# microsoft/M3P

Hardware: AMD Instinct MI355X
Metric: pre-train samples/sec (whole node), 12L/768d seq=128+36 (higher is better)
Workload: dtype bf16; 1 GPU; cfg2: 12L/768d/12h, 36 regions + 128 tokens, V=250002, 19 MLM targets/seq + ITM BCE, dropout 0.10, adam_inverse_sqrt + clip 5; per_gpu_batch=256, global_batch=256, seq_len=164, parallelism=dp1, prewarm_steps=36

## Files before the change

include/m3p_hip.h:

```cpp
#ifndef M3P_HIP_H
#define M3P_HIP_H

#include <stddef.h>
#include <stdint.h>

#ifdef __cplusplus
extern "C" {
#endif

#define M3P_API __attribute__((visibility("default")))

#define M3P_OK 0
#define M3P_EINVAL (-1)
#define M3P_ENOTIMPL (-2)
#define M3P_ENOMEM (-3)

M3P_API const char* m3p_version(void);


enum {
  M3P_EPI_NONE = 0,
  M3P_EPI_BIAS = 1,
  M3P_EPI_BIAS_GELU = 2,
  M3P_EPI_BIAS_DROP_RES = 3,
// ... 36 lines not shown
                            int M, int N, int K, int epilogue, const M3PEpilogue* ep, void* stream);

M3P_API int m3p_quant_fp8(const void* src, int ld_src, void* dst, int ld_dst, int rows, int cols, const float* scale,
                          float* amax, int bf8, void* stream);

M3P_API int m3p_quant_fp8_batch(const long long* desc, int n_desc, int blocks_per_matrix, void* stream);

M3P_API int m3p_gemm_nt_streamk_f32(const void* A, int lda, const void* W, int ldw, float* C, int ldc,
                                    int M, int N, int K, float alpha, void* stream);
M3P_API int m3p_gemm_nn_streamk_f32(const void* A, int lda, const void* W, int ldw, int k_valid, float* C,
                                    int ldc, int M, int N, int K, float alpha, void* stream);
M3P_API int m3p_gemm_nn_w4_f32(const void* A, int lda, const void* W, int ldw, float* C, int ldc, int M, int N, int K, float alpha,
                               void* workspace, size_t workspace_bytes, void* stream);

M3P_API size_t m3p_gemm_wgrad_workspace_bytes(void);
M3P_API int m3p_gemm_wgrad_bf16(const void* dY, int lddy, const void* X, int ldx, float* dW, int lddw,
                                int M, int N, int K, float alpha, void* workspace, size_t workspace_bytes,
                                void* stream);
M3P_API int m3p_gemm_wgrad_store_bf16(const void* dY, int lddy, const void* X, int ldx, float* dW, int lddw, int M, int N, int K,
                                      float alpha, void* workspace, size_t workspace_bytes, void* stream);
M3P_API int m3p_gemm_wgrad_pair_bf16(const void* dYa, int lddya, const void* Xa, int ldxa, float* dWa, int lddwa, int Na, int Ka,
                                     const void* dYb, int lddyb, const void* Xb, int ldxb, float* dWb, int lddwb, int Nb, int Kb,
                                     int M, float alpha, void* workspace, size_t workspace_bytes, void* stream);


M3P_API int m3p_layernorm_fwd(const void* x, const float* gamma, const float* beta, const uint8_t* rowmask,
                              void* y, float* mean, float* rstd, int rows, int d, float eps, void* stream);

M3P_API int m3p_layernorm_bwd(const void* dy_a, const void* dy_b, const void* x, const float* gamma,
                              const float* mean, const float* rstd, const uint8_t* rowmask,
                              void* dx, void* dx_drop, float* dgamma, float* dbeta, float* dbias_drop,
                              int rows, int d, uint32_t seed, uint32_t thresh24, float inv_keep, void* stream);
M3P_API int m3p_layernorm_bwd_rows(const void* dy_a, const void* dy_b, const void* x, const float* gamma,
                                   const float* mean, const float* rstd, const uint8_t* rowmask,
                                   void* dx, void* dx_drop, float* dgamma, float* dbeta, float* dbias_drop,
                                   int rows, int d, uint32_t seed, uint32_t thresh24, float inv_keep,
                                   const int32_t* rng_rows, void* stream);


M3P_API int m3p_attn_fwd(const void* qkv, const int32_t* keylen, void* ctx, float* lse, uint64_t* keepmask,
                         int B, int S, int H, int dh, uint32_t seed, uint32_t thresh24, float inv_keep,
                         void* stream);

M3P_API int m3p_attn_bwd(const void* qkv, const int32_t* keylen, const void* ctx, const void* dctx,
                         const float* lse, const uint64_t* keepmask, void* dqkv, float* dbias_qkv, int B, int S,
                         int H, int dh, float qscale, uint32_t seed, uint32_t thresh24, float inv_keep,
// ... 194 lines not shown
```

m3p_amd/csrc/gemm.hip:

```cpp
#include <mutex>
#include <type_traits>
#include "common.hpp"
#include "../../include/m3p_hip.h"
#include <hip/amd_detail/amd_hip_unsafe_atomics.h>

static int g_variant = 1;
extern "C" void m3p_debug_set_variant(int v) { g_variant = (v == 2 || v == 6) ? v : 1; }

namespace {

constexpr int BK = 64;
constexpr int ROWB = BK * 2;

#define M3P_DSR(dst, addr, off) asm volatile("ds_read_b128 %0, %1 offset:" #off : "=v"(dst) : "v"(addr))
#define M3P_TR(dst, addr, off) asm volatile("ds_read_b64_tr_b16 %0, %1 offset:" #off : "=v"(dst) : "v"(addr))
#define M3P_WAIT_LGKM(N) do { __builtin_amdgcn_sched_barrier(0); asm volatile("s_waitcnt lgkmcnt(" #N ")" ::: "memory"); __builtin_amdgcn_sched_barrier(0); } while (0)
#define M3P_WAIT_VM(N) do { __builtin_amdgcn_sched_barrier(0); asm volatile("s_waitcnt vmcnt(" #N ")" ::: "memory"); __builtin_amdgcn_sched_barrier(0); } while (0)
#define M3P_BAR() do { __builtin_amdgcn_s_barrier(); asm volatile("" ::: "memory"); __builtin_amdgcn_sched_barrier(0); } while (0)

__device__ __forceinline__ int xcd_slot(int nwg) {
  const int per_xcd = nwg >> 3;
  return (blockIdx.x & 7) * per_xcd + (blockIdx.x >> 3);
}
__device__ __forceinline__ int strip_width(int tiles_n, int from, int width) {
// ... 1647 lines not shown
      }
#pragma unroll
      for (int i = 0; i < 8; ++i)
#pragma unroll
        for (int j = 0; j < 4; ++j) acc[i][j] = f32x4{0.f, 0.f, 0.f, 0.f};
      if (more1) {
        read_w(nxt * STAGE, fw);
        read_a(Q0{}, nxt * STAGE, fa0);
        M3P_WAIT_LGKM(0);
      }
    }
  }
  if ((EPI == M3P_EPI_DGELU || EPI == M3P_EPI_MUL) && ep.colsum && csum_nw >= 0) flush_csum();
}


struct WgCursor {
  int c, t, mt, len;
};
struct WgradProblem {
  const bf16* dY; const bf16* X; float* dW;
  int lddy, ldx, lddw, tiles_i, tiles_j;
};

template <bool W_KN>
__global__ __launch_bounds__(512)
void gemm_nt_streamk_kernel(const bf16* __restrict__ A, int lda, const bf16* __restrict__ W, int ldw,
                            float* __restrict__ Cf, int ldc, int M, int N, int K, float alpha,
                            int tiles_m, int tiles_n, int CHUNK, int k_valid) {
  constexpr int BM = 256, BN = 128, NWAVES = 8;
  constexpr int A_BYTES = BM * ROWB, B_BYTES = BN * ROWB, STAGE = A_BYTES + B_BYTES;
  extern __shared__ __attribute__((aligned(16))) char smem[];
  const int tid = threadIdx.x, lane = tid & 63;
  const int wid = __builtin_amdgcn_readfirstlane(tid >> 6);
  const int ntile = tiles_m * tiles_n;
  const int nk = K / BK;
  const long long total_all = (long long)ntile * nk;
  const int nwg = gridDim.x;
  const int slot = xcd_slot(nwg);
  const long long share = (total_all + nwg - 1) / nwg;
  const long long g0l = share * slot;
  if (g0l >= total_all) return;
  const int total = (int)((g0l + share <= total_all ? g0l + share : total_all) - g0l);

  auto locate = [&](long long g) {
    WgCursor cu;
// ... 885 lines not shown
    return M3P_ENOTIMPL;
  return launch_wgrad_w4<true>(A, lda, W, ldw, C, ldc, K, M, N, alpha, workspace, workspace_bytes, stream, nullptr);
}

int m3p_gemm_wgrad_pair_bf16(const void* dYa, int lddya, const void* Xa, int ldxa, float* dWa, int lddwa, int Na, int Ka,
                             const void* dYb, int lddyb, const void* Xb, int ldxb, float* dWb, int lddwb, int Nb, int Kb,
                             int M, float alpha, void* workspace, size_t workspace_bytes, void* stream) {
  if (M <= 0 || Na <= 0 || Ka <= 0 || Nb <= 0 || Kb <= 0) return M3P_EINVAL;
  const bool pair = wgrad_w4_ok(M, Na, Ka, lddya, ldxa, dYa, Xa) && wgrad_w4_ok(M, Nb, Kb, lddyb, ldxb, dYb, Xb) &&
                    workspace && workspace_bytes >= m3p_gemm_wgrad_workspace_bytes() && (((uintptr_t)workspace & 15) == 0) &&
                    (lddwa % 4) == 0 && (lddwb % 4) == 0 && (((uintptr_t)dWa | (uintptr_t)dWb) & 15) == 0 &&
                    lddwa >= Ka && lddwb >= Kb &&
                    (long long)((Na / 256) * (Ka / 256) + (Nb / 256) * (Kb / 256)) * 2 <= num_cus();
  if (!pair) {
    int rc = m3p_gemm_wgrad_bf16(dYa, lddya, Xa, ldxa, dWa, lddwa, M, Na, Ka, alpha, workspace, workspace_bytes, stream);
    if (rc != M3P_OK) return rc;
    return m3p_gemm_wgrad_bf16(dYb, lddyb, Xb, ldxb, dWb, lddwb, M, Nb, Kb, alpha, workspace, workspace_bytes, stream);
  }
  if (lddya < Na || ldxa < Ka || lddyb < Nb || ldxb < Kb) return M3P_EINVAL;
  WgradProblem pb = {(const bf16*)dYb, (const bf16*)Xb, dWb, lddyb, ldxb, lddwb, Nb / 256, Kb / 256};
  return launch_wgrad_w4<>(dYa, lddya, Xa, ldxa, dWa, lddwa, M, Na, Ka, alpha, workspace, workspace_bytes, stream, &pb);
}

int m3p_gemm_wgrad_store_bf16(const void* dY, int lddy, const void* X, int ldx, float* dW, int lddw, int M, int N, int K,
                              float alpha, void* workspace, size_t workspace_bytes, void* stream) {
  if (M <= 0 || N <= 0 || K <= 0 || (lddy % 8) != 0 || (ldx % 8) != 0 || !dW || lddw < K) return M3P_EINVAL;
  if (lddy < N || ldx < K || ((uintptr_t)dY & 15) || ((uintptr_t)X & 15)) return M3P_EINVAL;
  if (!wgrad_w4_ok(M, N, K, lddy, ldx, dY, X)) return M3P_ENOTIMPL;
  return launch_wgrad_w4<>(dY, lddy, X, ldx, dW, lddw, M, N, K, alpha, workspace, workspace_bytes, stream, nullptr, true);
}

int m3p_gemm_wgrad_bf16(const void* dY, int lddy, const void* X, int ldx, float* dW, int lddw, int M, int N, int K,
                        float alpha, void* workspace, size_t workspace_bytes, void* stream) {
  if (M <= 0 || N <= 0 || K <= 0 || (lddy % 8) != 0 || (ldx % 8) != 0 || !dW || lddw < K) return M3P_EINVAL;
  if (lddy < ((N + 7) / 8) * 8 || ldx < ((K + 7) / 8) * 8) return M3P_EINVAL;
  if (((uintptr_t)dY & 15) || ((uintptr_t)X & 15)) return M3P_EINVAL;
  const int plan = wgrad_plan(M, N, K, wgrad_w4_ok(M, N, K, lddy, ldx, dY, X));
  if (plan == M3P_KERN_WGRAD_W4_CHUNKS || plan == M3P_KERN_WGRAD_W4_TILES) {
    return launch_wgrad_w4<>(dY, lddy, X, ldx, dW, lddw, M, N, K, alpha, workspace, workspace_bytes, stream, nullptr);
  }
  if (plan == M3P_KERN_WGRAD_RING) {
    const int ti = (N + WR_I - 1) / WR_I, tj = (K + WR_J - 1) / WR_J;
    const size_t lds = 3 * WR_STAGE;
    if (int rc = set_max_lds<gemm_wgrad_ring_kernel>(lds)) return rc;
    const int grid = num_cus();
    const int nmt = M / BK;
// ... 26 lines not shown
```

m3p_amd/csrc/gemm_wgrad_w4.hpp:

```cpp
template <bool YROWS>
__global__ __launch_bounds__(256)
void gemm_wgrad_w4_kernel(const bf16* __restrict__ dY_a, int lddy_a, const bf16* __restrict__ X_a, int ldx_a,
                          float* __restrict__ dW_a, int lddw_a, int M, int N, int K, float alpha,
                          int tiles_i, int tiles_j_a, int WR_CHUNK, float* __restrict__ ws, int* __restrict__ ws_tile,
                          int overwrite, WgradProblem pb) {
  const bf16* dY = dY_a;
  const bf16* X = X_a;
  float* dW = dW_a;
  int lddy = lddy_a, ldx = ldx_a, lddw = lddw_a, tiles_j = tiles_j_a;
  int tile_id0 = 0;
  constexpr int TI = 256, TJ = 256, KT = 64;
  constexpr int ROWB = 512;
  constexpr int Y_BYTES = KT * ROWB, STAGE = 2 * Y_BYTES;
  extern __shared__ __attribute__((aligned(16))) char smem[];
  const int tid = threadIdx.x, lane = tid & 63;
  const int wid = __builtin_amdgcn_readfirstlane(tid >> 6);
  const int ntile_a = tiles_i * tiles_j_a;
  const int ntile = ntile_a + pb.tiles_i * pb.tiles_j;
  const int nmt = M / KT;
  const long long total_all = (long long)ntile * nmt;
  const int nwg = gridDim.x;
  const int slot = xcd_slot(nwg);
  const bool rr = (WR_CHUNK == 0);
  if (ws && tid == 0) ws_tile[slot] = -1;
  int total, seg_tile, seg_m0, seg_len;
  if (rr) {
    const int my_tiles = (ntile > slot) ? (ntile - slot + nwg - 1) / nwg : 0;
    if (my_tiles == 0) return;
    total = my_tiles * nmt;
    seg_tile = slot; seg_m0 = 0; seg_len = nmt;
  } else {
    const int C = max(nwg / ntile, 1);
    if (slot >= C * ntile) return;
    const int c = slot / ntile;
    seg_tile = slot - c * ntile;
    if (seg_tile >= ntile_a) {
      dY = pb.dY; X = pb.X; dW = pb.dW; lddy = pb.lddy; ldx = pb.ldx; lddw = pb.lddw; tiles_j = pb.tiles_j;
      seg_tile -= ntile_a;
      tile_id0 = ntile_a;
    }
    seg_m0 = (int)((long long)c * nmt / C);
    seg_len = (int)((long long)(c + 1) * nmt / C) - seg_m0;
    total = seg_len;
    if (total <= 0) return;
  }
  (void)total_all;
  auto locate = [&](int) {
    WgCursor cu;
    cu.c = 0; cu.t = seg_tile; cu.mt = 0; cu.len = seg_len;
// ... 128 lines not shown
  asm volatile("" ::: "memory");
#pragma unroll
  for (int c = 0; c < 8; ++c) {
    WG_YRD(c, 0, 0);
    WG_TR2(xl[c], xh[c], x_addr[0][c], 0);
  }
  M3P_WAIT_LGKM(0);
#pragma unroll
  for (int c = 0; c < 8; ++c) { yf0[c] = yfrag(c); xf0[c] = frag(xl[c], xh[c]); }

  WgCursor cc = locate(g0);
  bool first = true;
  int n_seg = 0;
  auto kstep = [&](auto stage_c, int step) {
    if (first) wktile(std::true_type{}, stage_c);
    else wktile(std::false_type{}, stage_c);
    first = false;

    const bool last_of_tile = (cc.mt + 1 == cc.len) || (step + 1 == total);
    if (last_of_tile) {
      asm volatile("s_nop 15\n\ts_nop 15" ::: "memory");
      const int ti = cc.t / tiles_j, tj = cc.t - ti * tiles_j;
      float* dbase = dW + (size_t)(ti * TI + wi * 128 + fg * 4) * lddw + tj * TJ + wj * 128 + ft;
      const bool to_ws = (ws != nullptr) && !rr && n_seg == 0 && (step + 1 == total);
      if (to_ws) {
        asm volatile("s_waitcnt vmcnt(0)" ::: "memory");
        __builtin_amdgcn_s_barrier();
        asm volatile("" ::: "memory");
      }
#pragma nounroll
      for (int bb = 0; bb < 8; ++bb) {
        const int b = to_ws ? bb : ((bb + slot) & 7);
        float v[32];
#define WG_RD8(B)                                                                                   \
  _Pragma("unroll") for (int q = 0; q < 32; ++q) v[q] = 0.f;                                        \
  asm volatile("v_accvgpr_read_b32 %0, a[(" #B ")*32+0]\n\tv_accvgpr_read_b32 %1, a[(" #B ")*32+1]\n\t"   \
               "v_accvgpr_read_b32 %2, a[(" #B ")*32+2]\n\tv_accvgpr_read_b32 %3, a[(" #B ")*32+3]\n\t"   \
               "v_accvgpr_read_b32 %4, a[(" #B ")*32+4]\n\tv_accvgpr_read_b32 %5, a[(" #B ")*32+5]\n\t"   \
               "v_accvgpr_read_b32 %6, a[(" #B ")*32+6]\n\tv_accvgpr_read_b32 %7, a[(" #B ")*32+7]"       \
               : "=v"(v[0]), "=v"(v[1]), "=v"(v[2]), "=v"(v[3]), "=v"(v[4]), "=v"(v[5]), "=v"(v[6]), "=v"(v[7]));   \
  asm volatile("v_accvgpr_read_b32 %0, a[(" #B ")*32+8]\n\tv_accvgpr_read_b32 %1, a[(" #B ")*32+9]\n\t"   \
               "v_accvgpr_read_b32 %2, a[(" #B ")*32+10]\n\tv_accvgpr_read_b32 %3, a[(" #B ")*32+11]\n\t" \
               "v_accvgpr_read_b32 %4, a[(" #B ")*32+12]\n\tv_accvgpr_read_b32 %5, a[(" #B ")*32+13]\n\t" \
               "v_accvgpr_read_b32 %6, a[(" #B ")*32+14]\n\tv_accvgpr_read_b32 %7, a[(" #B ")*32+15]"     \
               : "=v"(v[8]), "=v"(v[9]), "=v"(v[10]), "=v"(v[11]), "=v"(v[12]), "=v"(v[13]), "=v"(v[14]), "=v"(v[15])); \
  asm volatile("v_accvgpr_read_b32 %0, a[(" #B ")*32+16]\n\tv_accvgpr_read_b32 %1, a[(" #B ")*32+17]\n\t" \
               "v_accvgpr_read_b32 %2, a[(" #B ")*32+18]\n\tv_accvgpr_read_b32 %3, a[(" #B ")*32+19]\n\t" \
// ... 4 lines not shown
               "v_accvgpr_read_b32 %2, a[(" #B ")*32+26]\n\tv_accvgpr_read_b32 %3, a[(" #B ")*32+27]\n\t" \
               "v_accvgpr_read_b32 %4, a[(" #B ")*32+28]\n\tv_accvgpr_read_b32 %5, a[(" #B ")*32+29]\n\t" \
               "v_accvgpr_read_b32 %6, a[(" #B ")*32+30]\n\tv_accvgpr_read_b32 %7, a[(" #B ")*32+31]"     \
               : "=v"(v[24]), "=v"(v[25]), "=v"(v[26]), "=v"(v[27]), "=v"(v[28]), "=v"(v[29]), "=v"(v[30]), "=v"(v[31]))
        switch (b) {
          case 0: { WG_RD8(0); } break;
          case 1: { WG_RD8(1); } break;
          case 2: { WG_RD8(2); } break;
          case 3: { WG_RD8(3); } break;
          case 4: { WG_RD8(4); } break;
          case 5: { WG_RD8(5); } break;
          case 6: { WG_RD8(6); } break;
          default: { WG_RD8(7); } break;
        }
#undef WG_RD8
        if (to_ws) {
          float* lw = reinterpret_cast<float*>(smem) + wid * (128 * 36) + (fg * 4) * 36 + (b & 1) * 16 + ft;
#pragma unroll
          for (int a = 0; a < 8; ++a)
#pragma unroll
            for (int r = 0; r < 4; ++r) lw[(a * 16 + r) * 36] = v[a * 4 + r];
          if (b & 1) {
            const float* lr = reinterpret_cast<const float*>(smem) + wid * (128 * 36) + (lane >> 3) * 36 + (lane & 7) * 4;
            float* wrow = ws + (size_t)slot * (TI * TJ + 272) + (size_t)(wi * 128 + (lane >> 3)) * TJ + wj * 128 + (b >> 1) * 32 + (lane & 7) * 4;
#pragma unroll
            for (int it = 0; it < 16; ++it)
              *reinterpret_cast<f32x4*>(wrow + it * 8 * TJ) = *reinterpret_cast<const f32x4*>(lr + it * 8 * 36);
          }
        } else {
          float* dcol = dbase + b * 16;
#pragma unroll
          for (int a = 0; a < 8; ++a)
#pragma unroll
            for (int r = 0; r < 4; ++r)
              if (overwrite) dcol[(size_t)(a * 16 + r) * lddw] = alpha * v[a * 4 + r];
              else unsafeAtomicAdd(dcol + (size_t)(a * 16 + r) * lddw, alpha * v[a * 4 + r]);
        }
      }
      if (to_ws && tid == 0) ws_tile[slot] = tile_id0 + cc.t;
      ++n_seg;
      first = true;
    }
    advance(cc);
  };
  for (int step = 0; step < total; step += 2) {
    kstep(std::integral_constant<int, 0>{}, step);
    if (step + 1 < total) kstep(std::integral_constant<int, 1>{}, step + 1);
  }
  asm volatile("s_waitcnt vmcnt(0)" ::: "memory");
#undef WG_LDB
#undef WG_TR2
#undef WG_YRD
#undef WG_ACC
#undef WG_M
#undef WG_L
}

__global__ __launch_bounds__(256)
void wgrad_reduce_kernel(const float* __restrict__ ws, const int* __restrict__ ws_tile, int nslots,
                         float* __restrict__ dW, int lddw, int tiles_j, float alpha, int ntile_a, WgradProblem pb) {
  const int t = blockIdx.y, rg = blockIdx.x;
  int tl = t;
// ... 26 lines not shown
```

m3p_amd/functional.py:

```python
import math
import os
from collections import OrderedDict

import torch

from . import lib as L
from . import fp8 as fp8mod
from . import ops
from . import rng

BF16 = torch.bfloat16
ALIGN = 64
BUCKET_ALIGN = 64 * 8


def _round_up(n, a):
    return (n + a - 1) // a * a


_VOCAB_FULL_TILES = os.environ.get('M3P_VOCAB_FULL_TILES', '1') != '0'
_GELU_GRAD_IN_FWD = os.environ.get('M3P_GELU_GRAD_IN_FWD', '0') != '0'
_GELU_BYTE_GRAD = int(os.environ.get('M3P_GELU_BYTE_GRAD', '2'))
_CE_FUSED_LSE = os.environ.get('M3P_CE_FUSED_LSE', '1') != '0'
_VOCAB_DGRAD_W4 = os.environ.get('M3P_VOCAB_DGRAD_W4', '1') != '0'
# ... 374 lines not shown

def first_rows_sink(model, tensor):
    d = model.dim
    if tensor.dim() != 3 or tensor.dtype != BF16 or not tensor._is_view():
        return None, None, None
    st, soff = tensor.stride(), tensor.storage_offset()
    if st[2] != 1 or st[0] % d or soff % d:
        return None, None, None
    with torch.no_grad():
        base = torch.as_strided(tensor, (tensor.untyped_storage().nbytes() // 2 // d, d), (d, 1), 0)
    sink = _sink_of(tensor, base)
    if sink is None:
        return None, None, None
    cache = model.__dict__.setdefault('_first_rows_cache', {})
    key = (tensor.shape[0], st[0], soff, tensor.device)
    rows = cache.get(key)
    if rows is None:
        rows = ((soff + torch.arange(tensor.shape[0], device=tensor.device, dtype=torch.int64) * st[0]) // d).to(torch.int32)
        cache.clear()
        cache[key] = rows
    return sink, base, rows


N_ENC_ARGS = 17

ROW_TILE = 256
COMPACT_MIN_ROWS = 4096


def compact_rows_eligible(n_rows, M):
    if n_rows <= 0:
        return 0
    n = _round_up(n_rows, ROW_TILE)
    return n if (n >= COMPACT_MIN_ROWS and 2 * n <= M) else 0


class OutputRows:

    def __init__(self, flags):
        flags = torch.as_tensor(flags).reshape(-1).cpu()
        if flags.dtype != torch.bool:
            flags = flags != 0
        self.flags = flags
        self.M = int(flags.numel())
        sel = torch.nonzero(flags).view(-1)
        self.n_rows = int(sel.numel())
# ... 225 lines not shown
        sunk = ctx.sink.take()
        if dout is None and sunk is None:
            if hook is not None:
                hook.encoder_backward_end()
            return (None,) * N_ENC_ARGS
        if dout is None:
            dh_ = sunk
        else:
            dh_ = dout.contiguous()
            if dh_.dtype != BF16:
                dh_ = dh_.to(BF16)
            if sunk is not None:
                dh_ = dh_ + sunk.view_as(dh_)
        last = hook.encoder_backward_begin() if hook is not None else True
        st8 = model.fp8_state() if model.fp8 else None

        def dgrad(g, i, gsite, wsite, wt16, epi, pre8=None, **kw):
            if st8 is None or wsite not in fp8mod.BWD_SITES:
                return ops.gemm_nt(g, wt16, epi, **kw)
            g8, dgs = pre8 if pre8 is not None else st8.quant(g, i, gsite)
            _, wt8, dws = st8.weights[(i, wsite)]
            return ops.gemm_nt_fp8(g8, wt8, epi, a_is_bf8=True, descale_a=dgs, descale_b=dws, **kw)

        for i in reversed(range(nL)):
            a, f = 'attentions.%d.' % i, 'ffns.%d.' % i
            (h_in, qkv, ctxt, lse, pre1, mean1, rstd1, x1, u, hact, pre2, mean2, rstd2, ctx_c, mask_i) = saved_layers[i]
            saved_layers[i] = None
            compact = rows_c is not None and i == nL - 1
            rr = {}
            if compact:
                rr = dict(rng_rows=rows_c.idx)
                dh_ = ops.gather_rows(dh_.view(M, d), rows_c.idx, rows_c.n, d)
            dpre2, dY2 = ops.layernorm_bwd(dh_, None, pre2, ar.p('layer_norm2.%d.weight' % i), mean2, rstd2, mask_i,
                                           ar.g('layer_norm2.%d.weight' % i), ar.g('layer_norm2.%d.bias' % i),
                                           dbias_drop=ar.g(f + 'lin2.bias'), want_drop=p_drop > 0,
                                           seed=seed('ffn', i), p_drop=p_drop, **rr)
            if dY2 is None:
                dY2 = dpre2
            ops.gemm_wgrad(dY2, hact, ar.g(f + 'lin2.weight'))
            du8 = None
            if ctx.u_holds_grad == 'q':
                o8 = {}
                if st8 is not None and 'w1' in fp8mod.BWD_SITES:
                    kd = st8.index(i, 'du')
                    if st8.seen[kd]:
                        o8 = dict(out8=torch.empty((M, 4 * d), dtype=torch.uint8, device=dY2.device), scale8=st8.scale[kd:kd + 1],
                                  amax8=st8.amax[kd:kd + 1], out8_bf8=True)
                dU = ops.gemm_nt(dY2, ar.wt[('lin2', i)], L.EPI_MULQ, aux=u, colsum=ar.g(f + 'lin1.bias'), **o8)
                if o8:
                    du8 = (o8['out8'], st8.descale[kd:kd + 1])
                elif st8 is not None and 'w1' in fp8mod.BWD_SITES:
                    st8._first_use(dU, kd)
            else:
                dU = dgrad(dY2, i, 'dy2', 'w2', ar.wt[('lin2', i)], L.EPI_MUL if ctx.u_holds_grad else L.EPI_DGELU, aux=u,
                           colsum=ar.g(f + 'lin1.bias'))
            del hact, u, pre2
            ops.gemm_wgrad(dU, x1, ar.g(f + 'lin1.weight'))
            dx1 = dgrad(dU, i, 'du', 'w1', ar.wt[('lin1', i)], L.EPI_RES, aux=dpre2, pre8=du8)
            del dU, dpre2, dY2
            dpre1, dAO = ops.layernorm_bwd(dx1, None, pre1, ar.p('layer_norm1.%d.weight' % i), mean1, rstd1, None,
                                           ar.g('layer_norm1.%d.weight' % i), ar.g('layer_norm1.%d.bias' % i),
                                           dbias_drop=ar.g(a + 'out_lin.bias'), want_drop=p_drop > 0,
                                           seed=seed('attn_out', i), p_drop=p_drop, **rr)
            if dAO is None:
                dAO = dpre1
            dctx = dgrad(dAO, i, 'dao', 'wout', ar.wt[('out', i)], L.EPI_NONE)
            if compact:
                ops.gemm_wgrad(dAO, ctx_c, ar.g(a + 'out_lin.weight'))
                dctx = ops.place_rows(dctx, rows_c.inv, M, 0)
                dpre1 = ops.place_rows(dpre1, rows_c.inv, M, 0)
            dqkv = ops.attn_bwd(qkv, totlen, ctxt, dctx, lse[0], B, S, H, dh, dbias_qkv=ar.qkv_bias(i, grad=True),
                                seed=seed('attn_p', i), p_drop=p_attn, keepmask=lse[1])
            if compact:
                ops.gemm_wgrad(dqkv, h_in, ar.qkv_wgrad(i))
            else:
                ops.gemm_wgrad_pair(dqkv, h_in, ar.qkv_wgrad(i), dAO, ctxt, ar.g(a + 'out_lin.weight'))
            dh_ = dgrad(dqkv, i, 'dqkv', 'wqkv', ar.wt[('qkv', i)], L.EPI_RES, aux=dpre1)
            del dqkv, dctx, dAO, dpre1, dx1
            ar.touch_layer(i)
            if hook is not None:
                hook.layer_done(i, last)
        if ctx.h0_mode is not None:
            if hook is not None:
                hook.embed_done(last, ids=None, rows=None, n_max=ctx.tok_rows_max)
            return (None,) * 14 + (dh_.to(ctx.h0_mode), None, None)
        want_dximg, has_text_embed = ctx.input_grads
        langs, positions = ctx.langs, ctx.positions
        tok_rows = None
        if has_text_embed or langs is not None or positions is not None or (hook is not None and hook.active):
            tok_rows = torch.empty((T * B, d), dtype=BF16, device=dh_.device)
        grads = dict(
            d_g_emb=ar.g('layer_norm_emb.weight'), d_be_emb=ar.g('layer_norm_emb.bias'),
            d_pos=ar.g('position_embeddings.weight'), d_emb=ar.g('embeddings.weight'),
            d_g_img=ar.g('image_embeddings.LayerNorm.weight'), d_be_img=ar.g('image_embeddings.LayerNorm.bias'),
            d_b_img=ar.g('image_embeddings.image_embeddings.bias'),
            d_b_loc=ar.g('image_embeddings.image_location_embeddings.bias'),
            d_w_loc=ar.g('image_embeddings.image_location_embeddings.weight'))
        de = ops.embed_assemble_bwd(dh_, emb_saved, ar.p('layer_norm_emb.weight'),
                                    ar.p('image_embeddings.LayerNorm.weight'), x, totlen, loc, grads, B, T, R, d,
                                    -1 if has_text_embed else model.pad_index, seed_img=seed('img'), seed_emb=seed('emb'), p_drop=p_drop,
                                    img_rows_bwd=None if ref_saved is None else
                                    (lambda g: refiner_bwd(model, g, ref_saved, keylen_img, B, R, seed_step, p_refine)),
                                    tok_rows=tok_rows)
        ar.touch('layer_norm_emb.weight', 'layer_norm_emb.bias', 'position_embeddings.weight')
# ... 725 lines not shown
```

m3p_amd/lib.py:

```python
import ctypes as C
import os

import torch

_HERE = os.path.dirname(os.path.abspath(__file__))
LIB_PATH = os.environ.get('M3P_HIP_LIB') or os.path.join(_HERE, 'libm3p_hip.so')

EPI_NONE, EPI_BIAS, EPI_BIAS_GELU, EPI_BIAS_DROP_RES, EPI_RES, EPI_DGELU, EPI_MUL, EPI_MULQ, EPI_BIAS_GELUQ, EPI_BIAS_LSE = range(10)
KERN_NT_SKINNY, KERN_NT_W8, KERN_NT_W8_QUEUE, KERN_NT_W4, KERN_NT_RING, KERN_NT_128 = range(1, 7)
KERN_WGRAD_W4_CHUNKS, KERN_WGRAD_W4_TILES, KERN_WGRAD_RING, KERN_WGRAD_128 = range(10, 14)


class M3PError(RuntimeError):
    pass


class Epilogue(C.Structure):
    _fields_ = [
        ('bias', C.c_void_p), ('aux', C.c_void_p), ('out2', C.c_void_p), ('colsum', C.c_void_p),
        ('ld_aux', C.c_int32), ('ld_out2', C.c_int32), ('scale_cols', C.c_int32), ('scale', C.c_float),
        ('alpha', C.c_float), ('seed', C.c_uint32), ('thresh24', C.c_uint32), ('inv_keep', C.c_float),
        ('descale_a', C.c_void_p), ('descale_b', C.c_void_p),
        ('out8', C.c_void_p), ('scale8', C.c_void_p), ('amax8', C.c_void_p), ('ld_out8', C.c_int32), ('out8_bf8', C.c_int32),
        ('rng_rows', C.c_void_p),
        ('row_ref', C.c_void_p),
    ]


_p, _i, _f, _u32 = C.c_void_p, C.c_int, C.c_float, C.c_uint32

SIGNATURES = {
    'm3p_version': (C.c_char_p, []),
    'm3p_gemm_nt_bf16': (_i, [_p, _i, _p, _i, _p, _i, _i, _i, _i, _i, C.POINTER(Epilogue), _p]),
    'm3p_gemm_nt_fp8': (_i, [_p, _i, _i, _p, _i, _p, _i, _i, _i, _i, _i, C.POINTER(Epilogue), _p]),
    'm3p_quant_fp8': (_i, [_p, _i, _p, _i, _i, _i, _p, _p, _i, _p]),
    'm3p_quant_fp8_batch': (_i, [_p, _i, _i, _p]),
    'm3p_gemm_nt_streamk_f32': (_i, [_p, _i, _p, _i, _p, _i, _i, _i, _i, _f, _p]),
    'm3p_gemm_nn_streamk_f32': (_i, [_p, _i, _p, _i, _i, _p, _i, _i, _i, _i, _f, _p]),
    'm3p_gemm_nn_w4_f32': (_i, [_p, _i, _p, _i, _p, _i, _i, _i, _i, _f, _p, C.c_size_t, _p]),
    'm3p_gemm_wgrad_workspace_bytes': (C.c_size_t, []),
    'm3p_gemm_wgrad_bf16': (_i, [_p, _i, _p, _i, _p, _i, _i, _i, _i, _f, _p, C.c_size_t, _p]),
    'm3p_gemm_wgrad_store_bf16': (_i, [_p, _i, _p, _i, _p, _i, _i, _i, _i, _f, _p, C.c_size_t, _p]),
    'm3p_gemm_wgrad_pair_bf16': (_i, [_p, _i, _p, _i, _p, _i, _i, _i, _p, _i, _p, _i, _p, _i, _i, _i, _i, _f, _p, C.c_size_t, _p]),
    'm3p_layernorm_fwd': (_i, [_p, _p, _p, _p, _p, _p, _p, _i, _i, _f, _p]),
    'm3p_layernorm_bwd': (_i, [_p, _p, _p, _p, _p, _p, _p, _p, _p, _p, _p, _p, _i, _i, _u32, _u32, _f, _p]),
    'm3p_layernorm_bwd_rows': (_i, [_p, _p, _p, _p, _p, _p, _p, _p, _p, _p, _p, _p, _i, _i, _u32, _u32, _f, _p, _p]),
    'm3p_attn_fwd': (_i, [_p, _p, _p, _p, _p, _i, _i, _i, _i, _u32, _u32, _f, _p]),
    'm3p_attn_bwd': (_i, [_p, _p, _p, _p, _p, _p, _p, _p, _i, _i, _i, _i, _f, _u32, _u32, _f, _p]),
    'm3p_attn_query_fwd': (_i, [_p, _i, _p, C.c_longlong, _i, _p, _p, _i, _i, _i, _i, _i, _i, _i, _p]),
    'm3p_attn_query_owner_fwd': (_i, [_p, _i, _p, C.c_longlong, _i, _p, _p, _i, _i, _i, _i, _i, _i, _i, _p, _i, _i, _p]),
    'm3p_vocab_select_max_k': (_i, []),
    'm3p_vocab_select_plan': (_i, [_i, _i, _i, _i, _i]),
    'm3p_vocab_select_workspace_bytes': (C.c_size_t, [_i, _i, _i]),
    'm3p_vocab_select': (_i, [_p, _i, _i, _i, _p, _i, _i, _p, C.c_size_t, _p, _p, _p, _p]),
    'm3p_vocab_sample_plan': (_i, [_i, _i, _i, _i]),
    'm3p_vocab_sample_workspace_bytes': (C.c_size_t, [_i, _i, _i]),
    'm3p_vocab_sample': (_i, [_p, _i, _i, _i, _f, _i, _u32, _p, C.c_size_t, _p, _p, _p, _p]),
    'm3p_attn_rows_fwd': (_i, [_p, _i, _p, C.c_longlong, _i, _p, _p, _p, _i, _i, _i, _i, _i, _i, _i, _u32, _u32, _f, _p]),
    'm3p_attn_rows_bwd': (_i, [_p, _i, _p, C.c_longlong, _i, _p, _p, _p, _p, _i, _p, _i, _i, _i, _i, _i, _i, _i, _f, _u32, _u32, _f, _p]),
    'm3p_attn_causal_fwd': (_i, [_p, _i, _p, _p, _i, _i, _i, _i, _u32, _u32, _f, _p]),
    'm3p_attn_causal_bwd': (_i, [_p, _i, _p, _p, _p, _i, _i, _i, _i, _i, _f, _u32, _u32, _f, _p]),
    'm3p_attn_cross_fwd': (_i, [_p, _i, _p, C.c_longlong, _i, _p, _p, _p, _i, _i, _i, _i, _i, _u32, _u32, _f, _p]),
    'm3p_attn_cross_bwd': (_i, [_p, _i, _p, C.c_longlong, _i, _p, _p, _p, _p, _i, _p, _i, _i, _i, _i, _i, _i, _f, _u32, _u32, _f, _p]),
    'm3p_cast_f32_bf16': (_i, [_p, _p, C.c_longlong, _p]),
    'm3p_embed_assemble_fwd': (_i, [_p] * 19 + [_i, _i, _i, _i, _u32, _u32, _u32, _f, _p, _p]),
    'm3p_embed_image_rows_fwd': (_i, [_p] * 10 + [_i, _i, _i, _u32, _u32, _f, _p]),
# ... 97 lines not shown
```

m3p_amd/ops.py:

```python
import ctypes as C
import os

import torch

from . import lib as L
from . import rng

BF16 = torch.bfloat16
_DEBUG_CHECKS = os.environ.get('M3P_DEBUG_CHECKS') == '1'

PROFILE = None
_EPI_NAMES = ['gemm_nt/none', 'gemm_nt/bias', 'gemm_nt/bias_gelu', 'gemm_nt/bias_drop_res', 'gemm_nt/res',
              'gemm_nt/dgelu', 'gemm_nt/mul', 'gemm_nt/mulq', 'gemm_nt/bias_geluq', 'gemm_nt/bias_lse']


PROFILE_ONLY = None


def _prof_begin(key=None):
    if PROFILE is None or (PROFILE_ONLY is not None and key != PROFILE_ONLY):
        return None
    e = torch.cuda.Event(enable_timing=True)
    e.record()
    return e
# ... 193 lines not shown
    rc = L.load().m3p_gemm_wgrad_bf16(dy.data_ptr(), dy.stride(0), x.data_ptr(), x.stride(0), dw.data_ptr(),
                                      dw.stride(0), M, N, K, alpha, ws.data_ptr(), ws.numel(), L.stream())
    L.check(rc, 'm3p_gemm_wgrad_bf16')
    _prof_end(e0, ('gemm_wgrad', M, N, K))
    return False if report_store else dw


def gemm_wgrad_pair(dy_a, x_a, dw_a, dy_b, x_b, dw_b, alpha=1.0):
    _chk_bf16(dy_a, x_a, dy_b, x_b)
    assert dw_a.dtype == torch.float32 and dw_b.dtype == torch.float32 and dw_a.stride(-1) == 1 and dw_b.stride(-1) == 1
    M = dy_a.shape[0]
    assert x_a.shape[0] == M and dy_b.shape[0] == M and x_b.shape[0] == M
    Na, Ka, Nb, Kb = dy_a.shape[1], x_a.shape[1], dy_b.shape[1], x_b.shape[1]
    assert dw_a.shape[0] >= Na and dw_a.shape[1] >= Ka and dw_b.shape[0] >= Nb and dw_b.shape[1] >= Kb
    e0 = _prof_begin(('gemm_wgrad_pair', M, Na + Nb, Ka))
    ws = _wgrad_workspace(dy_a.device)
    rc = L.load().m3p_gemm_wgrad_pair_bf16(dy_a.data_ptr(), dy_a.stride(0), x_a.data_ptr(), x_a.stride(0), dw_a.data_ptr(), dw_a.stride(0),
                                           Na, Ka, dy_b.data_ptr(), dy_b.stride(0), x_b.data_ptr(), x_b.stride(0), dw_b.data_ptr(),
                                           dw_b.stride(0), Nb, Kb, M, alpha, ws.data_ptr(), ws.numel(), L.stream())
    L.check(rc, 'm3p_gemm_wgrad_pair_bf16')
    _prof_end(e0, ('gemm_wgrad_pair', M, Na + Nb, Ka))


def layernorm_fwd(x, gamma, beta, rowmask=None, eps=1e-12):
    _chk_bf16(x)
    rows, d = x.shape
    assert x.is_contiguous()
    y = torch.empty_like(x)
    mean = torch.empty(rows, dtype=torch.float32, device=x.device)
    rstd = torch.empty(rows, dtype=torch.float32, device=x.device)
    rc = L.load().m3p_layernorm_fwd(x.data_ptr(), gamma.data_ptr(), beta.data_ptr(), L.ptr(rowmask), y.data_ptr(),
                                    mean.data_ptr(), rstd.data_ptr(), rows, d, eps, L.stream())
    L.check(rc, 'm3p_layernorm_fwd')
    return y, mean, rstd


def layernorm_bwd(dy_a, dy_b, x, gamma, mean, rstd, rowmask, dgamma, dbeta, dbias_drop=None,
                  want_drop=False, seed=0, p_drop=0.0, rng_rows=None):
    _chk_bf16(dy_a, dy_b, x)
    rows, d = x.shape
    if rng_rows is not None:
        assert rng_rows.dtype == torch.int32 and rng_rows.is_cuda and rng_rows.is_contiguous() and rng_rows.numel() == rows
    dx = torch.empty_like(x)
    dx_drop = torch.empty_like(x) if want_drop else None
    rc = L.load().m3p_layernorm_bwd_rows(dy_a.data_ptr(), L.ptr(dy_b), x.data_ptr(), gamma.data_ptr(), mean.data_ptr(),
                                         rstd.data_ptr(), L.ptr(rowmask), dx.data_ptr(), L.ptr(dx_drop),
# ... 732 lines not shown
```

Baseline: 8082 sequences/s.

## Batch weight-gradient GEMMs across layers into one grouped XCD-placed launch

Adds a grouped wgrad kernel path that queues several weight-gradient GEMMs (lin2, lin1, qkv, out_lin) from consecutive layers and runs them as one launch. Each workgroup owns one full 256x256 output tile and reduces over all of M, accumulating straight into dW with a read-modify-write. A host-side placement assigns tiles to XCDs so tiles of the same item share a die. This removes per-GEMM launch overhead, the split-M workspace reduction, and the atomics, and aims to fill all CUs at once. In exchange each workgroup does a long serial reduction, and the wgrad work is deferred and bunched later in the backward pass.

```diff
diff --git a/include/m3p_hip.h b/include/m3p_hip.h
--- a/include/m3p_hip.h
+++ b/include/m3p_hip.h
@@ -82,6 +82,13 @@
 M3P_API int m3p_gemm_wgrad_pair_bf16(const void* dYa, int lddya, const void* Xa, int ldxa, float* dWa, int lddwa, int Na, int Ka,
                                      const void* dYb, int lddyb, const void* Xb, int ldxb, float* dWb, int lddwb, int Nb, int Kb,
                                      int M, float alpha, void* workspace, size_t workspace_bytes, void* stream);
+#define M3P_WGRAD_GROUP_MAX 12
+typedef struct M3PWgradItem {
+  const void* dY; const void* X; float* dW;
+  int lddy, ldx, lddw, N, K;
+} M3PWgradItem;
+M3P_API int m3p_gemm_wgrad_group_bf16(const M3PWgradItem* items, int n_items, int M, float alpha, void* stream);
+M3P_API int m3p_gemm_wgrad_group_place(const int* tiles_i, const int* tiles_j, int n_items, int workgroups, uint32_t* place);
 
 
 M3P_API int m3p_layernorm_fwd(const void* x, const float* gamma, const float* beta, const uint8_t* rowmask,
diff --git a/m3p_amd/csrc/gemm.hip b/m3p_amd/csrc/gemm.hip
--- a/m3p_amd/csrc/gemm.hip
+++ b/m3p_amd/csrc/gemm.hip
@@ -1693,6 +1693,14 @@
   const bf16* dY; const bf16* X; float* dW;
   int lddy, ldx, lddw, tiles_i, tiles_j;
 };
+struct WgradGroup {
+  struct Item {
+    const bf16* dY; const bf16* X; float* dW;
+    int lddy, ldx, lddw, tiles_j;
+  } item[M3P_WGRAD_GROUP_MAX];
+  uint32_t place[256];
+};
+__device__ __forceinline__ const WgradGroup& wgrad_group_of(const WgradGroup& g) { return g; }
 
 template <bool W_KN>
 __global__ __launch_bounds__(512)
@@ -2624,6 +2632,77 @@
   return launch_wgrad_w4<>(dYa, lddya, Xa, ldxa, dWa, lddwa, M, Na, Ka, alpha, workspace, workspace_bytes, stream, &pb);
 }
 
+int m3p_gemm_wgrad_group_place(const int* tiles_i, const int* tiles_j, int n_items, int workgroups, uint32_t* place) {
+  if (!tiles_i || !tiles_j || !place || n_items < 1 || n_items > M3P_WGRAD_GROUP_MAX || workgroups < 8 || workgroups > 256 ||
+      (workgroups % 8) != 0)
+    return M3P_EINVAL;
+  const int per_xcd = workgroups / 8;
+  int total = 0;
+  for (int k = 0; k < n_items; ++k) {
+    if (tiles_i[k] < 1 || tiles_j[k] < 1 || tiles_i[k] > 256 || tiles_j[k] > 256) return M3P_EINVAL;
+    total += tiles_i[k] * tiles_j[k];
+    if (total > workgroups) return M3P_ENOTIMPL;
+  }
+  int used[8] = {0, 0, 0, 0, 0, 0, 0, 0};
+  int next[M3P_WGRAD_GROUP_MAX];
+  for (int w = 0; w < workgroups; ++w) place[w] = 0xffffffffu;
+  auto put = [&](int k, int xcd, int n) {
+    for (int e = 0; e < n; ++e, ++next[k], ++used[xcd])
+      place[used[xcd] * 8 + xcd] = (uint32_t)k << 16 | (uint32_t)(next[k] / tiles_j[k]) << 8 | (uint32_t)(next[k] % tiles_j[k]);
+  };
+  int xcd = 0;
+  for (int k = 0; k < n_items; ++k) {
+    next[k] = 0;
+    for (int full = tiles_i[k] * tiles_j[k] / per_xcd; full > 0; --full) put(k, xcd++, per_xcd);
+  }
+  int order[M3P_WGRAD_GROUP_MAX];
+  for (int k = 0; k < n_items; ++k) order[k] = k;
+  auto left = [&](int k) { return tiles_i[k] * tiles_j[k] - next[k]; };
+  std::stable_sort(order, order + n_items, [&](int a, int b) { return left(a) > left(b); });
+  for (int o = 0; o < n_items; ++o) {
+    const int k = order[o];
+    while (left(k) > 0) {
+      int best = -1, emptiest = 0;
+      for (int x = 0; x < 8; ++x) {
+        const int room = per_xcd - used[x];
+        if (room >= left(k) && (best < 0 || room < per_xcd - used[best])) best = x;
+        if (room > per_xcd - used[emptiest]) emptiest = x;
+      }
+      if (best >= 0) put(k, best, left(k));
+      else put(k, emptiest, per_xcd - used[emptiest]);
+    }
+  }
+  return M3P_OK;
+}
+
+int m3p_gemm_wgrad_group_bf16(const M3PWgradItem* items, int n_items, int M, float alpha, void* stream) {
+  if (!items || n_items < 1 || n_items > M3P_WGRAD_GROUP_MAX || M <= 0) return M3P_EINVAL;
+  const int grid = num_cus();
+  if (grid > 256) return M3P_ENOTIMPL;
+  WgradGroup grp;
+  int ti[M3P_WGRAD_GROUP_MAX], tj[M3P_WGRAD_GROUP_MAX];
+  for (int k = 0; k < n_items; ++k) {
+    const M3PWgradItem& it = items[k];
+    if (!it.dY || !it.X || !it.dW || it.N <= 0 || it.K <= 0) return M3P_EINVAL;
+    if (!wgrad_w4_ok(M, it.N, it.K, it.lddy, it.ldx, it.dY, it.X) || it.lddy < it.N || it.ldx < it.K || it.lddw < it.K ||
+        (it.lddw % 4) != 0 || ((uintptr_t)it.dW & 15) || it.N / 256 > 256 || it.K / 256 > 256)
+      return M3P_ENOTIMPL;
+    ti[k] = it.N / 256;
+    tj[k] = it.K / 256;
+    grp.item[k] = {(const bf16*)it.dY, (const bf16*)it.X, it.dW, it.lddy, it.ldx, it.lddw, tj[k]};
+  }
+  for (int k = n_items; k < M3P_WGRAD_GROUP_MAX; ++k) grp.item[k] = {nullptr, nullptr, nullptr, 0, 0, 0, 0};
+  for (int w = grid; w < 256; ++w) grp.place[w] = 0xffffffffu;
+  if (int rc = m3p_gemm_wgrad_group_place(ti, tj, n_items, grid, grp.place)) return rc;
+  const size_t lds = 2 * 65536;
+  if (int rc = set_max_lds<gemm_wgrad_w4_kernel<false, WgradGroup>>(lds)) return rc;
+  hipLaunchKernelGGL((gemm_wgrad_w4_kernel<false, WgradGroup>), dim3(grid), dim3(256), lds, (hipStream_t)stream,
+                     (const bf16*)nullptr, 0, (const bf16*)nullptr, 0, (float*)nullptr, 0, M, 0, 0, alpha, 0, 0, 1,
+                     (float*)nullptr, (int*)nullptr, 0, WgradProblem{}, grp);
+  M3P_CHECK_LAUNCH();
+  return M3P_OK;
+}
+
 int m3p_gemm_wgrad_store_bf16(const void* dY, int lddy, const void* X, int ldx, float* dW, int lddw, int M, int N, int K,
                               float alpha, void* workspace, size_t workspace_bytes, void* stream) {
   if (M <= 0 || N <= 0 || K <= 0 || (lddy % 8) != 0 || (ldx % 8) != 0 || !dW || lddw < K) return M3P_EINVAL;
diff --git a/m3p_amd/csrc/gemm_wgrad_w4.hpp b/m3p_amd/csrc/gemm_wgrad_w4.hpp
--- a/m3p_amd/csrc/gemm_wgrad_w4.hpp
+++ b/m3p_amd/csrc/gemm_wgrad_w4.hpp
@@ -1,9 +1,10 @@
-template <bool YROWS>
+template <bool YROWS, typename... GRP>
 __global__ __launch_bounds__(256)
 void gemm_wgrad_w4_kernel(const bf16* __restrict__ dY_a, int lddy_a, const bf16* __restrict__ X_a, int ldx_a,
                           float* __restrict__ dW_a, int lddw_a, int M, int N, int K, float alpha,
                           int tiles_i, int tiles_j_a, int WR_CHUNK, float* __restrict__ ws, int* __restrict__ ws_tile,
-                          int overwrite, WgradProblem pb) {
+                          int overwrite, WgradProblem pb, GRP... grp) {
+  constexpr bool GROUP = sizeof...(GRP) != 0;
   const bf16* dY = dY_a;
   const bf16* X = X_a;
   float* dW = dW_a;
@@ -21,10 +22,19 @@
   const long long total_all = (long long)ntile * nmt;
   const int nwg = gridDim.x;
   const int slot = xcd_slot(nwg);
-  const bool rr = (WR_CHUNK == 0);
-  if (ws && tid == 0) ws_tile[slot] = -1;
+  const bool rr = !GROUP && (WR_CHUNK == 0);
+  if (!GROUP && ws && tid == 0) ws_tile[slot] = -1;
   int total, seg_tile, seg_m0, seg_len;
-  if (rr) {
+  if constexpr (GROUP) {
+    const WgradGroup& g = wgrad_group_of(grp...);
+    const uint32_t pl = g.place[blockIdx.x];
+    if (pl == 0xffffffffu) return;
+    const WgradGroup::Item& it = g.item[pl >> 16];
+    dY = it.dY; X = it.X; dW = it.dW; lddy = it.lddy; ldx = it.ldx; lddw = it.lddw; tiles_j = it.tiles_j;
+    seg_tile = (int)((pl >> 8) & 255u) * tiles_j + (int)(pl & 255u);
+    seg_m0 = 0; seg_len = nmt;
+    total = nmt;
+  } else if (rr) {
     const int my_tiles = (ntile > slot) ? (ntile - slot + nwg - 1) / nwg : 0;
     if (my_tiles == 0) return;
     total = my_tiles * nmt;
@@ -199,7 +209,7 @@
       asm volatile("s_nop 15\n\ts_nop 15" ::: "memory");
       const int ti = cc.t / tiles_j, tj = cc.t - ti * tiles_j;
       float* dbase = dW + (size_t)(ti * TI + wi * 128 + fg * 4) * lddw + tj * TJ + wj * 128 + ft;
-      const bool to_ws = (ws != nullptr) && !rr && n_seg == 0 && (step + 1 == total);
+      const bool to_ws = GROUP || ((ws != nullptr) && !rr && n_seg == 0 && (step + 1 == total));
       if (to_ws) {
         asm volatile("s_waitcnt vmcnt(0)" ::: "memory");
         __builtin_amdgcn_s_barrier();
@@ -250,10 +260,20 @@
             for (int r = 0; r < 4; ++r) lw[(a * 16 + r) * 36] = v[a * 4 + r];
           if (b & 1) {
             const float* lr = reinterpret_cast<const float*>(smem) + wid * (128 * 36) + (lane >> 3) * 36 + (lane & 7) * 4;
+            if constexpr (GROUP) {
+              float* drow = dW + (size_t)(ti * TI + wi * 128 + (lane >> 3)) * lddw + tj * TJ + wj * 128 + (b >> 1) * 32 + (lane & 7) * 4;
+              f32x4 dv[16];
+#pragma unroll
+              for (int it = 0; it < 16; ++it) dv[it] = *reinterpret_cast<const f32x4*>(drow + (size_t)(it * 8) * lddw);
+#pragma unroll
+              for (int it = 0; it < 16; ++it)
+                *reinterpret_cast<f32x4*>(drow + (size_t)(it * 8) * lddw) = dv[it] + alpha * *reinterpret_cast<const f32x4*>(lr + it * 8 * 36);
+            } else {
             float* wrow = ws + (size_t)slot * (TI * TJ + 272) + (size_t)(wi * 128 + (lane >> 3)) * TJ + wj * 128 + (b >> 1) * 32 + (lane & 7) * 4;
 #pragma unroll
             for (int it = 0; it < 16; ++it)
               *reinterpret_cast<f32x4*>(wrow + it * 8 * TJ) = *reinterpret_cast<const f32x4*>(lr + it * 8 * 36);
+            }
           }
         } else {
           float* dcol = dbase + b * 16;
@@ -265,7 +285,7 @@
               else unsafeAtomicAdd(dcol + (size_t)(a * 16 + r) * lddw, alpha * v[a * 4 + r]);
         }
       }
-      if (to_ws && tid == 0) ws_tile[slot] = tile_id0 + cc.t;
+      if (!GROUP && to_ws && tid == 0) ws_tile[slot] = tile_id0 + cc.t;
       ++n_seg;
       first = true;
     }
diff --git a/m3p_amd/functional.py b/m3p_amd/functional.py
--- a/m3p_amd/functional.py
+++ b/m3p_amd/functional.py
@@ -420,6 +420,44 @@
     return sink, base, rows
 
 
+WGRAD_QUEUE_TILES = None
+
+
+class WgradQueue:
+    FILL = 7 / 8
+
+    def __init__(self, enabled=True):
+        self.capacity = 0 if not enabled else WGRAD_QUEUE_TILES if WGRAD_QUEUE_TILES is not None else L.num_cus()
+        self.units, self.tiles, self.items, self.M = [], 0, 0, None
+
+    @staticmethod
+    def _run(unit):
+        if len(unit) == 2:
+            ops.gemm_wgrad_pair(*unit[0], *unit[1])
+        else:
+            ops.gemm_wgrad(*unit[0])
+
+    def add(self, *unit):
+        M = unit[0][0].shape[0]
+        tiles = sum((dy.shape[1] // 256) * (x.shape[1] // 256) for dy, x, _ in unit)
+        if self.capacity <= 0 or tiles > self.capacity or not all(ops.wgrad_group_takes(*p) for p in unit):
+            self._run(unit)
+            return
+        if self.units and (M != self.M or self.tiles + tiles > self.capacity or self.items + len(unit) > L.WGRAD_GROUP_MAX):
+            self.flush()
+        self.units.append(unit)
+        self.tiles, self.items, self.M = self.tiles + tiles, self.items + len(unit), M
+
+    def flush(self):
+        units, tiles = self.units, self.tiles
+        self.units, self.tiles, self.items, self.M = [], 0, 0, None
+        if not units:
+            return
+        if tiles < self.FILL * self.capacity or not ops.gemm_wgrad_group([p for u in units for p in u]):
+            for u in units:
+                self._run(u)
+
+
 N_ENC_ARGS = 17
 
 ROW_TILE = 256
@@ -691,6 +729,7 @@
             _, wt8, dws = st8.weights[(i, wsite)]
             return ops.gemm_nt_fp8(g8, wt8, epi, a_is_bf8=True, descale_a=dgs, descale_b=dws, **kw)
 
+        wq = WgradQueue(enabled=hook is None and model.ddp_hook is None and st8 is None)
         for i in reversed(range(nL)):
             a, f = 'attentions.%d.' % i, 'ffns.%d.' % i
             (h_in, qkv, ctxt, lse, pre1, mean1, rstd1, x1, u, hact, pre2, mean2, rstd2, ctx_c, mask_i) = saved_layers[i]
@@ -706,7 +745,10 @@
                                            seed=seed('ffn', i), p_drop=p_drop, **rr)
             if dY2 is None:
                 dY2 = dpre2
-            ops.gemm_wgrad(dY2, hact, ar.g(f + 'lin2.weight'))
+            if compact:
+                ops.gemm_wgrad(dY2, hact, ar.g(f + 'lin2.weight'))
+            else:
+                wq.add((dY2, hact, ar.g(f + 'lin2.weight')))
             du8 = None
             if ctx.u_holds_grad == 'q':
                 o8 = {}
@@ -724,7 +766,10 @@
                 dU = dgrad(dY2, i, 'dy2', 'w2', ar.wt[('lin2', i)], L.EPI_MUL if ctx.u_holds_grad else L.EPI_DGELU, aux=u,
                            colsum=ar.g(f + 'lin1.bias'))
             del hact, u, pre2
-            ops.gemm_wgrad(dU, x1, ar.g(f + 'lin1.weight'))
+            if compact:
+                ops.gemm_wgrad(dU, x1, ar.g(f + 'lin1.weight'))
+            else:
+                wq.add((dU, x1, ar.g(f + 'lin1.weight')))
             dx1 = dgrad(dU, i, 'du', 'w1', ar.wt[('lin1', i)], L.EPI_RES, aux=dpre2, pre8=du8)
             del dU, dpre2, dY2
             dpre1, dAO = ops.layernorm_bwd(dx1, None, pre1, ar.p('layer_norm1.%d.weight' % i), mean1, rstd1, None,
@@ -743,12 +788,13 @@
             if compact:
                 ops.gemm_wgrad(dqkv, h_in, ar.qkv_wgrad(i))
             else:
-                ops.gemm_wgrad_pair(dqkv, h_in, ar.qkv_wgrad(i), dAO, ctxt, ar.g(a + 'out_lin.weight'))
+                wq.add((dqkv, h_in, ar.qkv_wgrad(i)), (dAO, ctxt, ar.g(a + 'out_lin.weight')))
             dh_ = dgrad(dqkv, i, 'dqkv', 'wqkv', ar.wt[('qkv', i)], L.EPI_RES, aux=dpre1)
             del dqkv, dctx, dAO, dpre1, dx1
             ar.touch_layer(i)
             if hook is not None:
                 hook.layer_done(i, last)
+        wq.flush()
         if ctx.h0_mode is not None:
             if hook is not None:
                 hook.embed_done(last, ids=None, rows=None, n_max=ctx.tok_rows_max)
diff --git a/m3p_amd/lib.py b/m3p_amd/lib.py
--- a/m3p_amd/lib.py
+++ b/m3p_amd/lib.py
@@ -27,6 +27,14 @@
     ]
 
 
+WGRAD_GROUP_MAX = 12
+
+
+class WgradItem(C.Structure):
+    _fields_ = [('dY', C.c_void_p), ('X', C.c_void_p), ('dW', C.c_void_p),
+                ('lddy', C.c_int32), ('ldx', C.c_int32), ('lddw', C.c_int32), ('N', C.c_int32), ('K', C.c_int32)]
+
+
 _p, _i, _f, _u32 = C.c_void_p, C.c_int, C.c_float, C.c_uint32
 
 SIGNATURES = {
@@ -42,6 +50,8 @@
     'm3p_gemm_wgrad_bf16': (_i, [_p, _i, _p, _i, _p, _i, _i, _i, _i, _f, _p, C.c_size_t, _p]),
     'm3p_gemm_wgrad_store_bf16': (_i, [_p, _i, _p, _i, _p, _i, _i, _i, _i, _f, _p, C.c_size_t, _p]),
     'm3p_gemm_wgrad_pair_bf16': (_i, [_p, _i, _p, _i, _p, _i, _i, _i, _p, _i, _p, _i, _p, _i, _i, _i, _i, _f, _p, C.c_size_t, _p]),
+    'm3p_gemm_wgrad_group_bf16': (_i, [C.POINTER(WgradItem), _i, _i, _f, _p]),
+    'm3p_gemm_wgrad_group_place': (_i, [C.POINTER(_i), C.POINTER(_i), _i, _i, C.POINTER(_u32)]),
     'm3p_layernorm_fwd': (_i, [_p, _p, _p, _p, _p, _p, _p, _i, _i, _f, _p]),
     'm3p_layernorm_bwd': (_i, [_p, _p, _p, _p, _p, _p, _p, _p, _p, _p, _p, _p, _i, _i, _u32, _u32, _f, _p]),
     'm3p_layernorm_bwd_rows': (_i, [_p, _p, _p, _p, _p, _p, _p, _p, _p, _p, _p, _p, _i, _i, _u32, _u32, _f, _p, _p]),
diff --git a/m3p_amd/ops.py b/m3p_amd/ops.py
--- a/m3p_amd/ops.py
+++ b/m3p_amd/ops.py
@@ -239,6 +239,44 @@
     _prof_end(e0, ('gemm_wgrad_pair', M, Na + Nb, Ka))
 
 
+def wgrad_group_takes(dy, x, dw):
+    M, N = dy.shape
+    K = x.shape[1]
+    return (M % 64 == 0 and M >= 4096 and N % 256 == 0 and K % 256 == 0 and dy.stride(1) == 1 and x.stride(1) == 1
+            and dw.stride(-1) == 1 and dy.stride(0) % 8 == 0 and x.stride(0) % 8 == 0 and dw.stride(0) % 4 == 0
+            and dw.stride(0) >= K and dy.data_ptr() % 16 == 0 and x.data_ptr() % 16 == 0 and dw.data_ptr() % 16 == 0)
+
+
+def wgrad_group_place(tiles, workgroups):
+    n = len(tiles)
+    ti = (C.c_int * n)(*[t[0] for t in tiles])
+    tj = (C.c_int * n)(*[t[1] for t in tiles])
+    place = (C.c_uint32 * max(workgroups, 1))()
+    L.check(L.load().m3p_gemm_wgrad_group_place(ti, tj, n, workgroups, place), 'm3p_gemm_wgrad_group_place')
+    return [None if p == 0xffffffff else (p >> 16, (p >> 8) & 255, p & 255) for p in place]
+
+
+def gemm_wgrad_group(items, alpha=1.0):
+    n = len(items)
+    assert 1 <= n <= L.WGRAD_GROUP_MAX
+    M = items[0][0].shape[0]
+    arr = (L.WgradItem * n)()
+    for k, (dy, x, dw) in enumerate(items):
+        _chk_bf16(dy, x)
+        assert dw.dtype == torch.float32 and dw.stride(-1) == 1 and dy.stride(1) == 1 and x.stride(1) == 1
+        assert dy.shape[0] == M and x.shape[0] == M and dw.shape[0] >= dy.shape[1] and dw.shape[1] >= x.shape[1]
+        arr[k] = L.WgradItem(dy.data_ptr(), x.data_ptr(), dw.data_ptr(), dy.stride(0), x.stride(0), dw.stride(0),
+                             dy.shape[1], x.shape[1])
+    key = ('gemm_wgrad_group', M, sum(dy.shape[1] * x.shape[1] for dy, x, _ in items) // 256, 256)
+    e0 = _prof_begin(key)
+    rc = L.load().m3p_gemm_wgrad_group_bf16(arr, n, M, alpha, L.stream())
+    if rc == -2:
+        return False
+    L.check(rc, 'm3p_gemm_wgrad_group_bf16')
+    _prof_end(e0, key)
+    return True
+
+
 def layernorm_fwd(x, gamma, beta, rowmask=None, eps=1e-12):
     _chk_bf16(x)
     rows, d = x.shape
```

Measured after the change: 8294 sequences/s (median of 6 runs). 1.03x the previous value.
